# diharaw/hybrid-rendering

Measured on AMD Instinct MI355X. Metric: shadow Mrays/s over the fully denoised frame (1 spp trace + SVGF temporal + 4x a-trous), higher is better.
Workload: dtype f32; 1 GPU; 1920x1080 procedural Sponza-like (277968 tris) ray-traced shadows 1spp + SVGF denoise; trace_launch_order=heaviest tiles of the last frame first (csrc/tile_order.h), rays_per_frame_per_gpu=729543, pixels_per_gpu=2073600, bvh_nodes=23425

## Files before the change

### hybrid_rendering_amd/csrc/denoise_fast_shadows.hip

```cpp
#include "denoise_fast_common.h"
#include "mask_window.h"
#include "tile_order.h"

namespace {

#ifndef FT_SHADOWS_EU
#define FT_SHADOWS_EU 6
#endif
template <int GEO, int PATHS>
__global__ __launch_bounds__(64 * FT_WAVES, FT_SHADOWS_EU) void kf_shadows_temporal(TemporalArgs a)
{
    if (geo_apron_rides<64 * FT_WAVES>(a.apron)) return;
    if (tile_order_rides<64 * FT_WAVES>(a.sort)) return;
    const uint2 BLK = block_xy<0>();
    __shared__ uint32_t s_mask[FT_WAVES][1][18];
    __shared__ MaskRows s_rows[FT_WAVES];
    const int  lane = threadIdx.x & 63, wave = threadIdx.x >> 6;
    const int  txr = BLK.x * FT_WAVES + wave;
    const bool tile_ok = txr < a.tiles_x;
    const int  tx = tile_ok ? txr : 0, ty = (int)BLK.y + a.tile_y0;
    const int  lx = lane & 7, ly = lane >> 3;
    const int  x = tx * 8 + lx, y = ty * 8 + ly;
    const bool in_image = tile_ok && x < a.w && y < a.h && y >= a.y0 && y < a.y1;
    const bool edge     = tile_ok && (x >= a.w || y >= a.h);
// ... 213 lines not shown
                const uint32_t so = (uint32_t)(py * a.w + px);
                const uint32_t s  = fm::ld<uint32_t>(a.in.p, so * 4u);
                const uint2    nd = fm::ld<uint2>(a.nd, so * 8u);
                sum.add(ek, cnz, cv, nz_of(nd.x, nd.y), s, kk, true);
            }
        result = sum.finish(a.power);
    }
    *outp = result;
    if (out2p) *out2p = result;
    return 1;
}

template <int STEP, bool N32>
__global__ __launch_bounds__(256) void kf_shadows_atrous(AtrousArgs a)
{
    (void)shadows_atrous_body<STEP, N32>(a);
}

template <int STEP>
__global__ __launch_bounds__(256) void kf_shadows_atrous_timeline(AtrousArgs a, unsigned long long* timeline)
{
    const AtrousTimeline tl;
    const int live = shadows_atrous_body<STEP, true>(a);
    tl.exit(timeline, live);
}


template <int STEP, bool N32>
__global__ __launch_bounds__(256) void kf_shadows_atrous_lds(AtrousArgs a)
{
    const uint2 BLK = block_xy<0>();
    constexpr int TW = 32 + 2 * STEP, TH = 8 + 2 * STEP;
    __shared__ uint32_t s_in[TH * TW];
    __shared__ float4   s_nz[TH * TW];
    const int lx = threadIdx.x & 31, ly = threadIdx.x >> 5;
    const int bx0 = (int)BLK.x * 32, by0 = a.y0 + (int)BLK.y * 8;
    if (bx0 >= a.w) return;
    const int x = bx0 + lx, y = by0 + ly;
    const bool inside = x < a.w && y < a.y1;
    const uint32_t cls = inside ? a.tile_class[(size_t)(y >> 3) * a.tiles_x + (x >> 3)] : 0u;
    if (__syncthreads_or((int)cls))
    {
        const int ry0 = a.y0 > 0 ? a.y0 : 0, ry1 = a.y1 < a.h ? a.y1 : a.h;
        ShadowsStageBatch<(TH * TW + 255) / 256, TW, TH * TW> batch;
        batch.load(a, bx0 - STEP, by0 - STEP, ry0, ry1);
        __builtin_amdgcn_sched_barrier(0);
        batch.store(s_in, s_nz);
        __syncthreads();
    }
    if (!inside) return;
    const uint32_t o = (uint32_t)(y * a.w + x);
    uint32_t* outp  = reinterpret_cast<uint32_t*>(reinterpret_cast<char*>(a.out) + o * 4u);
    uint32_t* out2p = a.out2 ? reinterpret_cast<uint32_t*>(reinterpret_cast<char*>(a.out2) + o * 4u) : nullptr;
    if (!cls)
    {
        *outp = 0u;
        if (out2p) *out2p = 0u;
        return;
    }
    const int      ci     = (ly + STEP) * TW + (lx + STEP);
    const uint32_t result = shadows_filter<true>(StagedTaps { s_in, s_nz, TW, ci, TW, ci, STEP }, [&] { return edge_setup(a.sigma_depth, a.phi_normal, N32); }, a.phi_visibility, a.power);
    *outp = result;
    if (out2p) *out2p = result;
}

template <int TH, bool N32>
HR_DEV int shadows_atrous01_body(const AtrousArgs& a, uint32_t* out_first2, float power1)
{
    const uint2 BLK = block_xy<0>();
    constexpr int AW = 38, AH = TH + 6, BW = 36, BH = TH + 4;
    __shared__ uint32_t s_in[AH * AW];
    __shared__ float4   s_nz[AH * AW];
    __shared__ uint32_t s_mid[BH * BW];
    const int bx0 = (int)BLK.x * 32, by0 = a.y0 + (int)BLK.y * TH;
    if (bx0 >= a.w) return 0;
    const int ry0 = a.y0 > 0 ? a.y0 : 0, ry1 = a.y1 < a.h ? a.y1 : a.h;
    uint32_t any_cls = 0u;
    {
        const uint32_t cols = a.tiles_x - (bx0 >> 3) >= 4 ? 0xffffffffu : (1u << ((a.tiles_x - (bx0 >> 3)) * 8)) - 1u;
#pragma unroll
        for (int r = 0; r < TH / 8; r++)
        {
            const bool      row  = by0 + 8 * r < ry1;
            const uint32_t  tb   = (uint32_t)((by0 >> 3) + (row ? r : 0)) * (uint32_t)a.tiles_x + (uint32_t)(bx0 >> 3);
            const uint32_t* tc   = reinterpret_cast<const uint32_t*>(a.tile_class) + (tb >> 2);
            const uint32_t  cls4 = (uint32_t)(((uint64_t)tc[0] | ((uint64_t)tc[1] << 32)) >> ((tb & 3u) * 8u));
            any_cls |= row ? (cls4 & cols) : 0u;
        }
    }
    if (!any_cls)
    {
        for (int j = threadIdx.x; j < TH * 32; j += 256)
        {
            const int x = bx0 + (j & 31), y = by0 + (j >> 5);
            if (x >= a.w || y >= a.y1) continue;
            const uint32_t o = (uint32_t)(y * a.w + x);
            a.out[o] = 0u;
            if (a.out2) a.out2[o] = 0u;
            if (out_first2) out_first2[o] = 0u;
        }
        return 0;
    }
    ShadowsStageBatch<(AH * AW + 255) / 256, AW, AH * AW> batch;
    batch.load(a, bx0 - 3, by0 - 3, ry0, ry1);
    __builtin_amdgcn_sched_barrier(0);
    batch.store(s_in, s_nz);
    __syncthreads();
    const EdgeK ek = edge_setup(a.sigma_depth, a.phi_normal, N32);
    auto filter = [&](const uint32_t* img, int IW, int vi, int ci, int D, float power) -> uint32_t {
        return shadows_filter<true>(StagedTaps { img, s_nz, IW, vi, AW, ci, D }, [&] { return ek; }, a.phi_visibility, power);
    };
    for (int j = threadIdx.x; j < BH * BW; j += 256)
    {
        const int  cy = j / BW, cx = j - cy * BW;
        const int  gx = bx0 - 2 + cx, gy = by0 - 2 + cy;
        const bool res = gx >= 0 && gx < a.w && gy >= ry0 && gy < ry1;
        uint32_t   r = 0u;
        if (res && a.tile_class[(size_t)(gy >> 3) * a.tiles_x + (gx >> 3)])
        {
            const int ci = (cy + 1) * AW + cx + 1;
            r = filter(s_in, AW, ci, ci, 1, 0.0f);
        }
        s_mid[j] = r;
        if (out_first2 && res && cx >= 2 && cx < 34 && cy >= 2 && cy < 2 + TH && gy < a.y1) out_first2[(uint32_t)(gy * a.w + gx)] = r;
    }
    __syncthreads();
    for (int j = threadIdx.x; j < TH * 32; j += 256)
    {
        const int lx = j & 31, ly = j >> 5, x = bx0 + lx, y = by0 + ly;
        if (x >= a.w || y >= a.y1) continue;
        const uint32_t o = (uint32_t)(y * a.w + x);
        uint32_t r = 0u;
        if (a.tile_class[(size_t)(y >> 3) * a.tiles_x + (x >> 3)]) r = filter(s_mid, BW, (ly + 2) * BW + lx + 2, (ly + 3) * AW + lx + 3, 2, power1);
        a.out[o] = r;
        if (a.out2) a.out2[o] = r;
    }
    return 1;
}

template <int TH, bool N32>
__global__ __launch_bounds__(256) void kf_shadows_atrous01(AtrousArgs a, uint32_t* out_first2, float power1)
{
    (void)shadows_atrous01_body<TH, N32>(a, out_first2, power1);
}

template <int TH>
__global__ __launch_bounds__(256) void kf_shadows_atrous01_timeline(AtrousArgs a, uint32_t* out_first2, float power1, unsigned long long* timeline)
{
    const AtrousTimeline tl;
    const int live = shadows_atrous01_body<TH, true>(a, out_first2, power1);
    tl.exit(timeline, live);
}

}

namespace hr {

void launch_shadows_temporal_fast(const TemporalArgs& a_, int n_tiles, hipStream_t st)
{
    TemporalArgs a = a_;
    const dim3 grid = grid_with_apron(grid_with_sort(a.sort, grid_cols(cdiv(a.tiles_x, FT_WAVES), 4), a.tiles_y), a.apron, 64 * FT_WAVES);
    if (!a.geo_hist) hipLaunchKernelGGL((kf_shadows_temporal<0, 0>), grid, dim3(64 * FT_WAVES), 0, st, a);
    else if ((a.paths & TP_PAIRS) && a.w >= 2) hipLaunchKernelGGL((kf_shadows_temporal<1, TP_PAIRS>), grid, dim3(64 * FT_WAVES), 0, st, a);
    else hipLaunchKernelGGL((kf_shadows_temporal<1, 0>), grid, dim3(64 * FT_WAVES), 0, st, a);
}

void launch_shadows_atrous_fast(const AtrousArgs& a, hipStream_t st, unsigned long long* timeline)
{
    const dim3 grid(grid_cols(cdiv(a.w, 32), a.step >= 4 ? 0 : 7), cdiv(a.y1 - a.y0, 8));
    const bool n32 = a.phi_normal == 32.0f;
    if (timeline && n32 && a.radius == 1 && (a.step == 4 || a.step == 8))
    {
        if (a.step == 4) hipLaunchKernelGGL((kf_shadows_atrous_timeline<4>), grid, dim3(256), 0, st, a, timeline);
        else hipLaunchKernelGGL((kf_shadows_atrous_timeline<8>), grid, dim3(256), 0, st, a, timeline);
        return;
    }
#define HR_LAUNCH_ATROUS(K, S) \
    do { if (n32) hipLaunchKernelGGL((K<S, true>), grid, dim3(256), 0, st, a); else hipLaunchKernelGGL((K<S, false>), grid, dim3(256), 0, st, a); } while (0)
    if (a.radius == 1 && a.step == 1) HR_LAUNCH_ATROUS(kf_shadows_atrous_lds, 1);
    else if (a.radius == 1 && a.step == 2) HR_LAUNCH_ATROUS(kf_shadows_atrous_lds, 2);
    else if (a.radius == 1 && a.step == 4) HR_LAUNCH_ATROUS(kf_shadows_atrous, 4);
    else if (a.radius == 1 && a.step == 8) HR_LAUNCH_ATROUS(kf_shadows_atrous, 8);
    else HR_LAUNCH_ATROUS(kf_shadows_atrous, 0);
#undef HR_LAUNCH_ATROUS
}

#ifndef FT_ATROUS01_TH
#define FT_ATROUS01_TH 16
#endif
bool launch_shadows_atrous01_fast(const AtrousArgs& a, uint32_t* out_first2, float power1, hipStream_t st, int lds_pad, unsigned long long* timeline)
{
    if (a.radius != 1 || a.step != 1) return false;
    const dim3   grid(grid_cols(cdiv(a.w, 32), 7), cdiv(a.y1 - a.y0, FT_ATROUS01_TH));
    const size_t pad = lds_pad > 0 ? (size_t)lds_pad : 0;
    if (a.phi_normal != 32.0f) hipLaunchKernelGGL((kf_shadows_atrous01<FT_ATROUS01_TH, false>), grid, dim3(256), pad, st, a, out_first2, power1);
    else if (timeline) hipLaunchKernelGGL((kf_shadows_atrous01_timeline<FT_ATROUS01_TH>), grid, dim3(256), pad, st, a, out_first2, power1, timeline);
    else hipLaunchKernelGGL((kf_shadows_atrous01<FT_ATROUS01_TH, true>), grid, dim3(256), pad, st, a, out_first2, power1);
    return true;
}

int shadows_atrous01_static_lds()
{
    hipFuncAttributes fa;
    if (hipFuncGetAttributes(&fa, reinterpret_cast<const void*>(&kf_shadows_atrous01<FT_ATROUS01_TH, true>)) != hipSuccess) { (void)hipGetLastError(); return -1; }
    return (int)fa.sharedSizeBytes;
}
int shadows_atrous_max_workgroups(const AtrousArgs& a)
{
    return (cdiv(a.w, 32) + 8) * cdiv(a.y1 - a.y0, 8);
}

}
```

### hybrid_rendering_amd/csrc/pass_args.h

```cpp
#pragma once
#include "reproject.h"
#include "shading.h"
#include "upsample.h"

namespace hr {

struct TileSortArgs
{
    const uint16_t* cost;
    uint32_t*       order;
    int             n, groups;
    int             row0;
    int             min_spread;
};

struct GeoApronArgs
{
    const void* gb2;
    const void* gb3;
    void*       out;
    int         w, a0, a1, b0, b1;
    int         row0;
};

struct TemporalArgs
{
    float           vpi[16];
    const uint32_t* mask;
    int             mw, mh;
    ImgRGBA16F      gb2, gb3, pgb2, pgb3;
    ImgR32F         depth, pdepth;
    ImgRG16F        hist;
    ImgRGBA16F      hist_moments;
    uint32_t*       out;
    uint2*          out_moments;
    uint8_t*        tile_class;
    float4*         nd;
    const void*     geo_hist;
    int             w, h, y0, y1;
    int             tiles_x, tiles_y, tile_y0;
    float           alpha, moments_alpha;
    int             debug_skip_reproject;
    uint32_t*       apron_flag;
    int             band_y0, band_y1;
    TileSortArgs    sort;
    GeoApronArgs    apron;
    int             paths;
};

enum TemporalPaths : int
{
    TP_PAIRS = 1,
    TP_ALL   = 1
};

struct AtrousArgs
{
    ImgRG16F       in;
    const float4*  nd;
    const uint8_t* tile_class;
    uint32_t*      out;
    uint32_t*      out2;
    int            w, h, y0, y1, tiles_x;
    int            radius, step;
    float          phi_visibility, phi_normal, sigma_depth, power;
};

struct AOTemporalArgs
{
    float           vpi[16];
    const uint32_t* mask;
    int             mw, mh, spp;
    ImgRGBA16F      gb2, gb3, pgb2, pgb3;
    ImgR32F         depth, pdepth;
    ImgR16F         hist, hist_len;
    uint16_t*       out;
    uint16_t*       out_len;
    uint8_t*        tile_class;
    const void*     geo_hist;
    void*           geo_out;
    int             geo_band;
    int             w, h, y0, y1;
    int             tiles_x, tiles_y, tile_y0;
    float           alpha;
    uint32_t*       apron_flag;
    int             band_y0, band_y1;
    TileSortArgs    sort;
};

struct AOBlurArgs
{
    ImgR16F        in;
    ImgR32F        depth;
    ImgRGBA16F     gb2;
    const uint8_t* tile_class;
    uint16_t*      out;
    float          zbp[4];
    int            w, h, y0, y1, tiles_x;
    int            dx, dy, radius;
};

struct ReflTemporalArgs
{
    float       vpi[16], pvp[16];
    float       cam[3];
    ImgRGBA16F  in, gb2, gb3, pgb2, pgb3, hist, hist_moments;
    ImgR32F     depth, pdepth;
    uint2*      out;
    uint2*      out_moments;
    uint8_t*    tile_class;
    const void* geo_hist;
    void*       geo_out;
    int         w, h, y0, y1, tiles_x;
    float       alpha, moments_alpha;
    int         approximate_with_ddgi, moving;
    uint32_t*   apron_flag;
    int         band_y0, band_y1;
    TileSortArgs sort;
};

struct ReflAtrousArgs
{
    ImgRGBA16F     in, gb2, gb3;
    ImgR32F        depth;
    const void*    geo;
    const uint8_t* tile_class;
    uint2*         out;
    uint2*         out2;
    int            w, h, y0, y1, tiles_x, radius, step;
    float          phi_color, phi_normal, sigma_depth;
    int            approximate_with_ddgi;
};

struct DDGISampleArgs
{
    DDGIU        d;
    float        vpi[16];
    float        cam[3];
    const float* depth;
    const uint2* gb2;
    AtlasRGBA    irr;
    AtlasRG      dep;
    uint2*       out;
    int          w, h, y0, y1;
    float        gi_intensity;
};

void launch_shadows_temporal_fast(const TemporalArgs& a, int n_tiles, hipStream_t st);
void launch_shadows_atrous_fast(const AtrousArgs& a, hipStream_t st, unsigned long long* timeline = nullptr);
bool launch_shadows_atrous01_fast(const AtrousArgs& a, uint32_t* out_first2, float power1, hipStream_t st, int lds_pad = 0, unsigned long long* timeline = nullptr);
int  shadows_atrous01_static_lds();
int  shadows_atrous_max_workgroups(const AtrousArgs& a);
void launch_ao_temporal_fast(const AOTemporalArgs& a, int n_tiles, hipStream_t st);
void launch_ao_blur_fast(const AOBlurArgs& a, hipStream_t st);
bool launch_ao_blur_xy_fast(const AOBlurArgs& a, hipStream_t st);
void launch_refl_temporal_fast(const ReflTemporalArgs& a, hipStream_t st);
void launch_refl_atrous_fast(const ReflAtrousArgs& a, hipStream_t st);
bool launch_refl_atrous01_fast(const ReflAtrousArgs& a, uint2* out_first2, hipStream_t st);
void launch_ddgi_sample_fast(const DDGISampleArgs& a, hipStream_t st);
void launch_upsample_fast(const UpsampleArgs& a, hipStream_t st);

}
```

### hybrid_rendering_amd/csrc/shadows.hip

```cpp
#include "hr_internal.h"
#include "reproject.h"
#include "traverse.h"
#include "traverse2.h"
#include "shading.h"
#include "cutout_host.h"
#include "upsample.h"
#include "pass_args.h"
#include "tile_order.h"
#include "pass_core.h"

using namespace hr;

struct TraceArgs
{
    float           vpi[16];
    hr_light        light;
    const float*    depth;
    const uint2*    gb2;
    const uint8_t*  sobol;
    const uint8_t*  sr;
    uint32_t*       mask;
    uint16_t*       ray_slots;
    const Node8*    nodes;
    const TriGPU*   tris;
// ... 200 lines not shown
            {
                float sv = max2(mean - mean * mean, 0.0f);
                float sd = hr_sqrt(sv);
                hv       = clamp1(hv, mean - 0.5f * sd, mean + 0.5f * sd);
            }
            const float al = success ? max2(a.alpha, __fdiv_rn(1.0f, hlen)) : 1.0f;
            const float am = success ? max2(a.moments_alpha, __fdiv_rn(1.0f, hlen)) : 1.0f;
            m0      = visibility;
            m1      = m0 * m0;
            m0      = mix1(hm[0], m0, am);
            m1      = mix1(hm[1], m1, am);
            out_var = max2(0.0f, m1 - m0 * m0);
            out_v   = mix1(hv, visibility, al);
            flag    = out_v > 0.0f;
        }
        if (in_image)
        {
            a.out_moments[pix] = make_uint2(pack_h2(m0, m1), pack_h2(hlen, 0.0f));
            a.nd[pix]  = make_float4(cn.x, cn.y, cn.z, h2f_hi(cg3.y));
            a.out[pix] = pack_h2(out_v, out_var);
        }
    }
    if (a.apron_flag && __ballot(apron_miss) && lane == 0) atomicOr(a.apron_flag, 1u);
    const unsigned long long any = __ballot(flag);
    if (lane == 0) a.tile_class[(size_t)ty * a.tiles_x + tx] = any ? 1 : 0;
}


template <bool FAST>
HR_DEV float edge_weight(float cd, float sd, float phi_z, f3 cn, f3 sn, float phi_n, float cl, float sl, const DivBy& phi_l)
{
    const float dz = -fabsf(cd - sd);
    const float wZ = det_exp(FAST ? dz : __fdiv_rn(dz, phi_z));
    const float dn = clamp1(dot3(cn, sn), 0.0f, 1.0f);
    float wN;
    if (FAST) { float b = dn * dn; b = b * b; b = b * b; b = b * b; wN = b * b; }
    else wN = det_pow_auto(dn, phi_n);
    const float wL = div_by(fabsf(cl - sl), phi_l);
    return det_exp((0.0f - max2(wL, 0.0f)) - max2(wZ, 0.0f)) * wN;
}

template <int RADIUS, bool FAST>
__global__ __launch_bounds__(256) void k_shadows_atrous(AtrousArgs a)
{
    const int x = blockIdx.x * 32 + (threadIdx.x & 31);
    const int y = a.y0 + blockIdx.y * 8 + (threadIdx.x >> 5);
    if (x >= a.w || y >= a.y1) return;
    const size_t o = (size_t)y * a.w + x;
    if (!a.tile_class[(size_t)(y >> 3) * a.tiles_x + (x >> 3)])
    {
        a.out[o] = 0u;
        if (a.out2) a.out2[o] = 0u;
        return;
    }
    const uint32_t c  = a.in.p[o];
    uint32_t t_in[8];
    float4   t_nd[8];
    bool     t_ok[8];
    if (RADIUS == 1)
    {
#pragma unroll
        for (int t = 0; t < 8; t++)
        {
            const int k = t < 4 ? t : t + 1, xx = k % 3 - 1, yy = k / 3 - 1;
            const int px = x + xx * a.step, py = y + yy * a.step;
            t_ok[t] = px >= 0 && py >= 0 && px < a.w && py < a.h;
            const bool res = t_ok[t] && py >= a.y0 && py < a.y1;
            t_in[t] = res ? a.in.p[(size_t)py * a.w + px] : 0u;
            t_nd[t] = res ? a.nd[(size_t)py * a.w + px] : make_float4(0.0f, 0.0f, 0.0f, 0.0f);
        }
    }
    const float    cv = h2f_lo(c);
    float var = 0.0f;
#pragma unroll
    for (int yy = -1; yy <= 1; yy++)
#pragma unroll
        for (int xx = -1; xx <= 1; xx++)
        {
            const float k = (xx == 0 ? (yy == 0 ? 0.25f : 0.125f) : (yy == 0 ? 0.125f : 0.0625f));
            var += h2f_hi(a.in.raw(x + xx, y + yy)) * k;
        }
    const float4 cnd = a.nd[o];
    const float center_depth = cnd.w;
    uint32_t    result;
    if (center_depth < 0.0f) result = c;
    else
    {
        const f3    cn    = mk3(cnd.x, cnd.y, cnd.z);
        const DivBy phi_v = div_prepare(a.phi_visibility * hr_sqrt(max2(0.0f, 1e-10f + var)));
        float sum_w = 1.0f, sum_v = cv, sum_var = h2f_hi(c);
        if (RADIUS == 1)
        {
            float w8[8];
#pragma unroll
            for (int t = 0; t < 8; t++)
                w8[t] = edge_weight<FAST>(center_depth, t_nd[t].w, a.sigma_depth, cn, mk3(t_nd[t].x, t_nd[t].y, t_nd[t].z), a.phi_normal, cv, h2f_lo(t_in[t]), phi_v);
#pragma unroll
            for (int t = 0; t < 8; t++)
            {
                if (!t_ok[t]) continue;
                const int   k = t < 4 ? t : t + 1, xx = k % 3 - 1, yy = k / 3 - 1;
                const float kx = xx == 0 ? 1.0f : __fdiv_rn(2.0f, 3.0f), ky = yy == 0 ? 1.0f : __fdiv_rn(2.0f, 3.0f);
                const float sv = h2f_lo(t_in[t]);
                const float wv = w8[t] * (kx * ky);
                sum_w += wv;
                sum_v += wv * sv;
                sum_var += (wv * wv) * h2f_hi(t_in[t]);
            }
        }
        else
        {
        const int R = RADIUS >= 0 ? RADIUS : a.radius;
        for (int yy = -R; yy <= R; yy++)
            for (int xx = -R; xx <= R; xx++)
            {
                const int px = x + xx * a.step, py = y + yy * a.step;
                if (px < 0 || py < 0 || px >= a.w || py >= a.h || (xx == 0 && yy == 0)) continue;
                const int   axx = xx < 0 ? -xx : xx, ayy = yy < 0 ? -yy : yy;
                const float kx = axx == 0 ? 1.0f : (axx == 1 ? __fdiv_rn(2.0f, 3.0f) : __fdiv_rn(1.0f, 6.0f));
                const float ky = ayy == 0 ? 1.0f : (ayy == 1 ? __fdiv_rn(2.0f, 3.0f) : __fdiv_rn(1.0f, 6.0f));
                const uint32_t s  = a.in.raw(px, py);
                const float4   snd = (py >= a.y0 && py < a.y1) ? a.nd[(size_t)py * a.w + px] : make_float4(0.0f, 0.0f, 0.0f, 0.0f);
                const float    sv = h2f_lo(s);
                const f3       sn = mk3(snd.x, snd.y, snd.z);
                const float    w  = edge_weight<FAST>(center_depth, snd.w, a.sigma_depth, cn, sn, a.phi_normal, cv, sv, phi_v);
                const float    wv = w * (kx * ky);
                sum_w += wv;
                sum_v += wv * sv;
                sum_var += (wv * wv) * h2f_hi(s);
            }
        }
        float ov = __fdiv_rn(sum_v, sum_w), ovar = __fdiv_rn(sum_var, sum_w * sum_w);
        if (a.power != 0.0f) ov = det_pow_auto(ov, a.power);
        result = pack_h2(ov, ovar);
    }
    a.out[o] = result;
    if (a.out2) a.out2[o] = result;
}

struct hr_shadows : PassCore
{
    DevBuf  mask, temporal_out, moments[2], prev_image, atrous[2], nd, occluder;
    int     temporal_paths = TP_ALL;
    bool    occluder_cache = true;
    int     read_idx = 0;
    int     last_ping_pong = 0;
    int           latched_exact = -1;
    int           dbg_only_tx = -1, dbg_only_ty = -1;
    bool          dbg_skip_traversal = false, dbg_skip_reproject = false, dbg_timeline_stats = false;
    std::string   dbg_timeline;
    uint64_t      last_wave_max_steps = 0;
    void*         nd_cur = nullptr;
    int           atrous01_pad = 0;
    std::string   dbg_atrous_timeline;
};

#ifndef FT_ATROUS01_RESIDENT
#define FT_ATROUS01_RESIDENT 6
#endif
#ifndef HR_ATROUS01_REGIONS_PER_SLOT
#define HR_ATROUS01_REGIONS_PER_SLOT 4
#endif
#define HR_LDS_GRANULE 1280

struct AtrousTimelineDump
{
    DevBuf buf;
    unsigned long long* ptr() const { return (unsigned long long*)buf.p; }
    hr_status begin(const std::string& prefix, const AtrousArgs& a)
    {
        if (prefix.empty()) return HR_OK;
        return buf.alloc((size_t)shadows_atrous_max_workgroups(a) * 4 * 32);
    }
    hr_status end(const std::string& prefix, const char* tag, hipStream_t st)
    {
        if (!buf.p) return HR_OK;
        HR_HIP(hipStreamSynchronize(st));
        std::vector<unsigned long long> host(buf.bytes / 8);
        HR_HIP(hipMemcpy(host.data(), buf.p, buf.bytes, hipMemcpyDeviceToHost));
        if (FILE* f = fopen((prefix + "." + tag).c_str(), "wb")) { fwrite(host.data(), 8, host.size(), f); fclose(f); }
        return HR_OK;
    }
};

bool hr::profiling_enabled(const hr_shadows* p) { return p && p->prof.enabled; }

extern "C" {

void hr_shadows_default_params(hr_shadows_params* p)
{
    p->denoise = 1; p->bias = 0.5f; p->alpha = 0.01f; p->moments_alpha = 0.2f; p->phi_visibility = 10.0f;
    p->phi_normal = 32.0f; p->sigma_depth = 1.0f; p->power = 1.2f; p->radius = 1; p->filter_iterations = 4; p->feedback_iteration = 1;
    p->exact = 1;
}

hr_status hr_shadows_create(hr_ctx* ctx, int32_t full_width, int32_t full_height, hr_scale scale, const hr_band* band, hr_shadows** out)
{
    hr_shadows* p = nullptr;
    hr_status   s = pass_new(&p, ctx, full_width, full_height, scale, band, out, BandRule::Shadows, "shadows");
    if (s != HR_OK) return s;
    if (const char* e = getenv("HR_DEBUG_ONLY_TILE")) sscanf(e, "%d,%d", &p->dbg_only_tx, &p->dbg_only_ty);
    if (const char* e = getenv("HR_SHADOW_CACHE")) p->occluder_cache = atoi(e) != 0;
    if (const char* e = getenv("HR_TEMPORAL_PAIRS")) p->temporal_paths = atoi(e) != 0 ? (p->temporal_paths | TP_PAIRS) : (p->temporal_paths & ~TP_PAIRS);
    p->tile_order.min_spread = HR_ORDER_COHERENT_SPREAD;
    p->dbg_skip_traversal = getenv("HR_DEBUG_SKIP_TRAVERSAL") != nullptr;
    p->dbg_skip_reproject = getenv("HR_DEBUG_SKIP_REPROJECT") != nullptr;
    p->dbg_timeline_stats = getenv("HR_DEBUG_TIMELINE_STATS") != nullptr;
    if (const char* e = getenv("HR_DEBUG_TIMELINE")) p->dbg_timeline = e;
    if (const char* e = getenv("HR_DEBUG_ATROUS_TIMELINE")) p->dbg_atrous_timeline = e;
    {
        int resident = FT_ATROUS01_RESIDENT;
        if (const char* e = getenv("HR_ATROUS01_RESIDENT")) resident = atoi(e);
        hipDeviceProp_t prop;
        if (resident >= 3 && hipGetDeviceProperties(&prop, ctx->device) == hipSuccess)
        {
            const int own = shadows_atrous01_static_lds(), regions = cdiv(p->w, 32) * cdiv(p->y1 - p->y0, 16);
            if (regions > HR_ATROUS01_REGIONS_PER_SLOT * resident * prop.multiProcessorCount) resident = 0;
            if (own >= 0) p->atrous01_pad = atrous_resident_pad((int)prop.maxSharedMemoryPerMultiProcessor, own, resident, HR_LDS_GRANULE);
            if (own + p->atrous01_pad > (int)prop.sharedMemPerBlock) p->atrous01_pad = 0;
        }
    }
    const size_t px = (size_t)p->w * p->h;
    HR_PASS_ALLOC(mask, (size_t)p->mw * p->mh * 4)
    HR_PASS_ALLOC(temporal_out, px * 4)
    HR_PASS_ALLOC(moments[0], px * 8)
    HR_PASS_ALLOC(moments[1], px * 8)
    HR_PASS_ALLOC(prev_image, px * 4)
    HR_PASS_ALLOC(atrous[0], px * 4)
    HR_PASS_ALLOC(atrous[1], px * 4)
    HR_PASS_ALLOC(upsample, (size_t)full_width * full_height * 2)
    HR_PASS_ALLOC(tile_class, (((size_t)p->tiles_x * p->tiles_y + 3) & ~(size_t)3) + 8)
    HR_PASS_ALLOC(nd, px * 16)
    HR_PASS_ALLOC(counters, 64)
    HR_PASS_ALLOC(ray_slots, (size_t)p->tiles_x * p->tiles_y * 2)
    HR_PASS_ALLOC(occluder, px * 4)
    if ((s = p->tile_order.init(p->resident_tiles())) != HR_OK) { delete p; return s; }
    HR_HIP(hipMemset(p->occluder.p, 0xff, p->occluder.bytes));
    HR_HIP(hipMemset(p->counters.p, 0, 64));
    HR_HIP(hipMemset(p->ray_slots.p, 0, p->ray_slots.bytes));
    HR_HIP(hipMemset(p->mask.p, 0, p->mask.bytes));
    HR_HIP(hipMemset(p->tile_class.p, 0, p->tile_class.bytes));
    *out = p;
    return HR_OK;
}

hr_status hr_shadows_destroy(hr_shadows* p) { return pass_destroy(p); }
hr_status hr_shadows_reset_history(hr_shadows* p) { return pass_reset_history(p); }
hr_status hr_shadows_history_apron_exceeded(hr_shadows* p, int32_t* exceeded) { return pass_history_apron_exceeded(p, exceeded); }
hr_status hr_shadows_set_profiling(hr_shadows* p, int32_t enable) { return pass_set_profiling(p, enable); }
hr_status hr_shadows_get_stage_times(hr_shadows* p, hr_stage_times* out) { return pass_get_stage_times(p, out); }
hr_status hr_shadows_ray_count(hr_shadows* p, uint64_t* rays) { return pass_ray_count<uint16_t>(p, rays); }
hr_status hr_shadows_launch_order(hr_shadows* p, uint32_t* out, int32_t* n_tiles) { return pass_launch_order(p, out, n_tiles); }

hr_status hr_shadows_tile_ray_counts(hr_shadows* p, uint16_t* out, int32_t* tiles_x, int32_t* tiles_y)
{
    HR_CHECK_ARG(p);
    if (tiles_x) *tiles_x = p->tiles_x;
    if (tiles_y) *tiles_y = p->tiles_y;
    if (!out) return HR_OK;
    HR_HIP(hipStreamSynchronize(p->last_stream));
    HR_HIP(hipMemcpy(out, p->ray_slots.p, (size_t)p->tiles_x * p->tiles_y * 2, hipMemcpyDeviceToHost));
    return HR_OK;
}

hr_status hr_shadows_ray_trace(hr_shadows* p, const hr_scene* scene, const hr_frame_inputs* in, const hr_shadows_params* prm, void* stream_)
{
    HR_CHECK_ARG(p && scene && in && prm);
    hr_status s = check_inputs(p, in, false);
    if (s != HR_OK) return s;
    HR_CHECK_ARG(in->sobol && in->scrambling_ranking);
    HR_REJECT_SHARED_DEV(scene, "hr_shadows_ray_trace", p->want_stats || !p->dbg_timeline.empty() || p->dbg_skip_traversal || p->dbg_only_tx >= 0);
    HR_REJECT_CUTOUT(scene, HR_RAY_SHADOW, "hr_shadows_ray_trace", p->want_stats || !p->dbg_timeline.empty() || p->dbg_skip_traversal || p->dbg_only_tx >= 0);
    const bool       cutout = cutout_on(scene, HR_RAY_SHADOW);
    const CutoutView cv = cutout ? cutout_view_of(scene) : CutoutView();
    hipStream_t st = (hipStream_t)stream_;
    p->last_stream = st;
    if (p->first_frame)
    {
        HR_HIP(hipMemsetAsync(p->prev_image.p, 0, p->prev_image.bytes, st));
        HR_HIP(hipMemsetAsync(p->moments[!in->ping_pong].p, 0, p->moments[0].bytes, st));
        p->first_frame = false;
    }
    TraceArgs a;
    for (int i = 0; i < 16; i++) a.vpi[i] = in->ubo.view_proj_inverse[i];
    a.light = in->ubo.light;
    a.depth = in->cur.depth; a.gb2 = (const uint2*)in->cur.gb2;
    a.sobol = in->sobol; a.sr = in->scrambling_ranking;
    a.mask = (uint32_t*)p->mask.p; a.ray_slots = (uint16_t*)p->ray_slots.p;
    a.nodes = (const Node8*)scene->nodes.p; a.tris = (const TriGPU*)scene->tris.p; a.inst = (const InstanceShared*)scene->inst_shared.p; a.cull = cull_of(scene, HR_RAY_SHADOW);
    a.stats = nullptr;
    a.timeline = nullptr;
    a.w = p->w; a.h = p->h; a.y0 = p->y0; a.y1 = p->y1; a.mw = p->mw;
    a.tile_y0 = p->tile_y0(); a.tiles_x = p->tiles_x; a.tiles_y = p->resident_tiles_y();
    a.bias = prm->bias; a.num_frames = in->num_frames;
    a.occluder = p->occluder_cache ? (uint32_t*)p->occluder.p : nullptr;
    a.n_tri_refs = (uint32_t)(scene->tris.bytes / sizeof(TriGPU));
    const int n_tiles = a.tiles_x * a.tiles_y;
    const int n_slots = n_tiles;
    a.debug_only_tx = p->dbg_only_tx; a.debug_only_ty = p->dbg_only_ty;
    a.debug_skip_traversal = p->dbg_skip_traversal ? 1 : 0;
    if ((s = p->tile_order.flush(st)) != HR_OK) return s;
    a.order = p->tile_order.order_arg(n_tiles); a.cost = p->tile_order.cost_arg(n_tiles);
    const uint64_t px = (uint64_t)p->w * (p->y1 - p->y0);
    if (p->want_stats)
    {
        a.cost = nullptr;
        HR_HIP(hipMemsetAsync((char*)p->counters.p + 16, 0, 24, st));
        a.stats = (unsigned long long*)((char*)p->counters.p + 16);
        hipLaunchKernelGGL(k_shadows_trace<true>, dim3(cdiv(n_slots, TRACE_WAVES)), dim3(64 * TRACE_WAVES), 0, st, a, cv);
        HR_HIP(hipGetLastError());
        return HR_OK;
    }
    if (!p->dbg_timeline.empty())
    {
        const char* tl = p->dbg_timeline.c_str();
        DevBuf buf;
        hr_status bs = buf.alloc((size_t)n_tiles * 32);
        if (bs != HR_OK) return bs;
        a.timeline = (unsigned long long*)buf.p;
        if (p->dbg_timeline_stats) hipLaunchKernelGGL(k_shadows_trace<true>, dim3(cdiv(n_slots, TRACE_WAVES)), dim3(64 * TRACE_WAVES), 0, st, a, cv);
        else hipLaunchKernelGGL(k_shadows_trace<false>, dim3(cdiv(n_slots, TRACE_WAVES)), dim3(64 * TRACE_WAVES), 0, st, a, cv);
        HR_HIP(hipStreamSynchronize(st));
        std::vector<unsigned long long> host((size_t)n_tiles * 4);
        HR_HIP(hipMemcpy(host.data(), buf.p, host.size() * 8, hipMemcpyDeviceToHost));
        if (FILE* f = fopen(tl, "wb")) { fwrite(host.data(), 8, host.size(), f); fclose(f); }
        a.timeline = nullptr;
    }
    int ev = p->prof.begin("ray_trace", st, px * 12 + px / 8);
    const auto kernel = scene->shared ? (cutout ? k_shadows_trace<false, true, true> : k_shadows_trace<false, true>)
                                      : (cutout ? k_shadows_trace<false, false, true> : k_shadows_trace<false>);
    hipLaunchKernelGGL(kernel, dim3(cdiv(n_slots, TRACE_WAVES)), dim3(64 * TRACE_WAVES), 0, st, a, cv);
    p->prof.end(ev, st);
    HR_HIP(hipGetLastError());
    if (a.cost && (s = p->tile_order.traced(n_tiles, st)) != HR_OK) return s;
    return HR_OK;
}

hr_status hr_shadows_trace_divergence(hr_shadows* p, uint64_t* wave_max_steps)
{
    HR_CHECK_ARG(p && wave_max_steps);
    *wave_max_steps = p->last_wave_max_steps;
    return HR_OK;
}

static hr_status shadows_trace_stats_impl(hr_shadows* p, const hr_scene* scene, const hr_frame_inputs* in, const hr_shadows_params* prm, uint64_t* out3, void* stream, bool walk_only)
{
    HR_CHECK_ARG(p && out3);
    const bool cache = p->occluder_cache;
    p->want_stats = true;
    if (walk_only) p->occluder_cache = false;
    hr_status s = hr_shadows_ray_trace(p, scene, in, prm, stream);
    p->want_stats = false;
    p->occluder_cache = cache;
    if (s != HR_OK) return s;
    HR_HIP(hipStreamSynchronize((hipStream_t)stream));
    uint64_t host[5];
    HR_HIP(hipMemcpy(host, p->counters.p, 40, hipMemcpyDeviceToHost));
    hr_status rs = hr_shadows_ray_count(p, &out3[0]);
    if (rs != HR_OK) return rs;
    out3[1] = host[2]; out3[2] = host[3];
    p->last_wave_max_steps = host[4];
    return HR_OK;
}

hr_status hr_shadows_trace_stats(hr_shadows* p, const hr_scene* scene, const hr_frame_inputs* in, const hr_shadows_params* prm, uint64_t* out3, void* stream)
{
    return shadows_trace_stats_impl(p, scene, in, prm, out3, stream, true);
}

hr_status hr_shadows_trace_stats_timed(hr_shadows* p, const hr_scene* scene, const hr_frame_inputs* in, const hr_shadows_params* prm, uint64_t* out3, void* stream)
{
    return shadows_trace_stats_impl(p, scene, in, prm, out3, stream, false);
}

hr_status hr_shadows_temporal(hr_shadows* p, const hr_frame_inputs* in, const hr_shadows_params* prm, void* stream_)
{
    HR_CHECK_ARG(p && in && prm);
    hr_status s = check_inputs(p, in, true);
    if (s != HR_OK) return s;
    hipStream_t st = (hipStream_t)stream_;
    p->last_stream = st;
    p->latched_exact = prm->exact ? 1 : 0;
    TemporalArgs a;
    for (int i = 0; i < 16; i++) a.vpi[i] = in->ubo.view_proj_inverse[i];
    a.mask = (const uint32_t*)p->mask.p; a.mw = p->mw; a.mh = p->mh;
    const int w = p->w, y0 = p->y0, y1 = p->y1, ry0 = p->ry0, ry1 = p->ry1;
    a.gb2  = ImgRGBA16F { (const uint2*)in->cur.gb2, w, ry0, ry1 };
    a.gb3  = ImgRGBA16F { (const uint2*)in->cur.gb3, w, ry0, ry1 };
    a.pgb2 = ImgRGBA16F { (const uint2*)in->prev.gb2, w, ry0, ry1 };
    a.pgb3 = ImgRGBA16F { (const uint2*)in->prev.gb3, w, ry0, ry1 };
    a.depth  = ImgR32F { in->cur.depth, w, ry0, ry1 };
    a.pdepth = ImgR32F { in->prev.depth, w, ry0, ry1 };
    a.hist         = ImgRG16F { (const uint32_t*)p->prev_image.p, w, ry0, ry1 };
    a.hist_moments = ImgRGBA16F { (const uint2*)p->moments[!in->ping_pong].p, w, ry0, ry1 };
    a.out = (uint32_t*)p->temporal_out.p; a.out_moments = (uint2*)p->moments[in->ping_pong ? 1 : 0].p;
    a.tile_class = (uint8_t*)p->tile_class.p;
    a.nd = (float4*)p->nd.p;
    a.geo_hist = nullptr;
    a.apron = GeoApronArgs { nullptr, nullptr, nullptr, 0, 0, 0, 0, 0, -1 };
    if (!prm->exact)
    {
        const size_t half = (size_t)p->w * p->h * 8;
        const GeoRecords::Step g = p->records.advance(in->cur.gb2, in->cur.gb3, in->prev.gb2, in->prev.gb3, p->first_frame);
        if (g.read >= 0) a.geo_hist = (const char*)p->nd.p + (size_t)g.read * half;
        a.nd = (float4*)((char*)p->nd.p + (size_t)g.write * half);
        if (p->records.history && (ry0 < y0 || ry1 > y1))
            a.apron = GeoApronArgs { in->cur.gb2, in->cur.gb3, a.nd, w, ry0, y0, y1, ry1, -1 };
        if (g.require_failed) return geo_require_error("hr_shadows_temporal");
    }
    else p->records.invalidate();
    p->nd_cur = a.nd;
    a.w = w; a.h = p->h; a.y0 = y0; a.y1 = y1;
    a.tile_y0 = p->tile_y0(); a.tiles_x = p->tiles_x; a.tiles_y = p->resident_tiles_y();
    a.alpha = prm->alpha; a.moments_alpha = prm->moments_alpha;
    a.debug_skip_reproject = p->dbg_skip_reproject ? 1 : 0;
    a.apron_flag = p->apron_flag();
    a.band_y0 = p->band_y0; a.band_y1 = p->band_y1;
    a.paths = p->temporal_paths;
    p->last_ping_pong = in->ping_pong ? 1 : 0;
    const uint64_t px = (uint64_t)w * (y1 - y0);
    int ev = p->prof.begin("temporal_accumulation", st, px * 64 + px / 8);
    a.sort = TileSortArgs { nullptr, nullptr, 0, 0, 0, 0 };
    if (prm->exact) hipLaunchKernelGGL(k_shadows_temporal, dim3(cdiv(a.tiles_x * a.tiles_y, TEMPORAL_WAVES)), dim3(64 * TEMPORAL_WAVES), 0, st, a);
    else
    {
        a.sort = p->tile_order.ride();
        launch_shadows_temporal_fast(a, a.tiles_x * a.tiles_y, st);
    }
    p->prof.end(ev, st);
    HR_HIP(hipGetLastError());
    return HR_OK;
}

static hr_status check_mode(hr_shadows* p, const hr_shadows_params* prm);

hr_status hr_shadows_atrous_iteration(hr_shadows* p, const hr_frame_inputs* in, const hr_shadows_params* prm, int32_t i, void* stream_)
{
    HR_CHECK_ARG(p && in && prm && i >= 0 && i < prm->filter_iterations && prm->filter_iterations <= 8 && prm->radius >= 0 && prm->radius <= 2);
    hr_status s = check_inputs(p, in, false);
    if (s != HR_OK) return s;
    if ((s = check_mode(p, prm)) != HR_OK) return s;
    hipStream_t st = (hipStream_t)stream_;
    p->last_stream = st;
    const int read_idx = i & 1, write_idx = (i & 1) ^ 1;
    AtrousArgs a;
    const int w = p->w, y0 = p->y0, y1 = p->y1;
    a.in  = ImgRG16F { (const uint32_t*)(i == 0 ? p->temporal_out.p : p->atrous[read_idx].p), w, y0, y1 };
    a.nd = (const float4*)(p->nd_cur ? p->nd_cur : p->nd.p);
    a.tile_class = (const uint8_t*)p->tile_class.p;
    a.out  = (uint32_t*)p->atrous[write_idx].p;
    a.out2 = (prm->feedback_iteration == i) ? (uint32_t*)p->prev_image.p : nullptr;
    a.w = w; a.h = p->h; a.y0 = y0; a.y1 = y1; a.tiles_x = p->tiles_x;
    a.radius = prm->radius; a.step = 1 << i;
    a.phi_visibility = prm->phi_visibility; a.phi_normal = prm->phi_normal; a.sigma_depth = prm->sigma_depth;
    a.power = (i == prm->filter_iterations - 1) ? prm->power : 0.0f;
    p->read_idx = write_idx;
    static const char* names[8] = { "atrous_0", "atrous_1", "atrous_2", "atrous_3", "atrous_4", "atrous_5", "atrous_6", "atrous_7" };
    const uint64_t px = (uint64_t)w * (y1 - y0);
    int ev = p->prof.begin(names[i], st, px * 24 + (a.out2 ? px * 4 : 0));
    const dim3 grid(cdiv(w, 32), cdiv(y1 - y0, 8));
    const bool fast = (prm->phi_normal == 32.0f && prm->sigma_depth == 1.0f);
    AtrousTimelineDump tl;
    if (!prm->exact && p->fuse && prm->radius == 1 && (i == 2 || i == 3) && (s = tl.begin(p->dbg_atrous_timeline, a)) != HR_OK) return s;
    if (!prm->exact) launch_shadows_atrous_fast(a, st, tl.ptr());
    else if (prm->radius == 1 && fast) hipLaunchKernelGGL((k_shadows_atrous<1, true>), grid, dim3(256), 0, st, a);
    else if (prm->radius == 1) hipLaunchKernelGGL((k_shadows_atrous<1, false>), grid, dim3(256), 0, st, a);
    else hipLaunchKernelGGL((k_shadows_atrous<-1, false>), grid, dim3(256), 0, st, a);
    p->prof.end(ev, st);
    HR_HIP(hipGetLastError());
    if ((s = tl.end(p->dbg_atrous_timeline, i == 2 ? "atrous4" : "atrous8", st)) != HR_OK) return s;
    return HR_OK;
}

static hr_status check_mode(hr_shadows* p, const hr_shadows_params* prm)
{
    if (p->latched_exact >= 0 && p->latched_exact != (prm->exact ? 1 : 0))
    {
        set_last_error("hr_shadows: params.exact changed between the temporal and the a-trous stage of one frame");
        return HR_ERR_INVALID_ARG;
    }
    return HR_OK;
}

static hr_status shadows_atrous01(hr_shadows* p, const hr_frame_inputs* in, const hr_shadows_params* prm, void* stream_, bool* done)
{
    hr_status s = check_inputs(p, in, false);
    if (s != HR_OK) return s;
    if ((s = check_mode(p, prm)) != HR_OK) return s;
    hipStream_t st = (hipStream_t)stream_;
    p->last_stream = st;
    AtrousArgs a;
    const int w = p->w, y0 = p->y0, y1 = p->y1;
    a.in  = ImgRG16F { (const uint32_t*)p->temporal_out.p, w, y0, y1 };
    a.nd = (const float4*)(p->nd_cur ? p->nd_cur : p->nd.p);
    a.tile_class = (const uint8_t*)p->tile_class.p;
    a.out  = (uint32_t*)p->atrous[0].p;
    a.out2 = (prm->feedback_iteration == 1) ? (uint32_t*)p->prev_image.p : nullptr;
    uint32_t* first2 = (prm->feedback_iteration == 0) ? (uint32_t*)p->prev_image.p : nullptr;
    a.w = w; a.h = p->h; a.y0 = y0; a.y1 = y1; a.tiles_x = p->tiles_x;
    a.radius = prm->radius; a.step = 1;
    a.phi_visibility = prm->phi_visibility; a.phi_normal = prm->phi_normal; a.sigma_depth = prm->sigma_depth;
    a.power = 0.0f;
    const uint64_t px = (uint64_t)w * (y1 - y0);
    AtrousTimelineDump tl;
    if ((s = tl.begin(p->dbg_atrous_timeline, a)) != HR_OK) return s;
    int ev = p->prof.begin("atrous_01", st, px * 16 + ((a.out2 || first2) ? px * 4 : 0));
    *done = launch_shadows_atrous01_fast(a, first2, prm->filter_iterations == 2 ? prm->power : 0.0f, st, p->atrous01_pad, tl.ptr());
    p->prof.end(ev, st);
    if ((s = tl.end(p->dbg_atrous_timeline, "atrous01", st)) != HR_OK) return s;
    if (*done) p->read_idx = 0;
    HR_HIP(hipGetLastError());
    return HR_OK;
}

hr_status hr_shadows_upsample(hr_shadows* p, const hr_frame_inputs* in, const hr_shadows_params* prm, void* stream)
{
    HR_CHECK_ARG(p && in && prm);
    const uint64_t PX = (uint64_t)p->full_w * p->full_h, px = (uint64_t)p->w * p->h;
    return pass_upsample(p, in, prm->exact != 0, p->atrous[p->read_idx].p, 2, 1, 0.0f, 0.0f, PX * 18 + px * 20, stream);
}

hr_status hr_shadows_denoise(hr_shadows* p, const hr_frame_inputs* in, const hr_shadows_params* prm, void* stream)
{
    HR_CHECK_ARG(p && in && prm);
    p->last_denoise = prm->denoise != 0;
    if (!prm->denoise) return HR_OK;
    hr_status s;
    if ((s = hr_shadows_temporal(p, in, prm, stream)) != HR_OK) return s;
    {
        HR_SCOPED_SAMPLE("A-Trous Filter");
        bool fused = false;
        if (!prm->exact && p->fuse && prm->filter_iterations >= 2 && prm->filter_iterations <= 8 && prm->radius == 1 &&
            (s = shadows_atrous01(p, in, prm, stream, &fused)) != HR_OK) return s;
        for (int i = fused ? 2 : 0; i < prm->filter_iterations; i++)
            if ((s = hr_shadows_atrous_iteration(p, in, prm, i, stream)) != HR_OK) return s;
    }
    if (p->scale != 0 && (s = hr_shadows_upsample(p, in, prm, stream)) != HR_OK) return s;
    return HR_OK;
}

hr_status hr_shadows_render(hr_shadows* p, const hr_scene* scene, const hr_frame_inputs* in, const hr_shadows_params* prm, void* stream)
{
    HR_SCOPED_SAMPLE("Ray Traced Shadows");
    HR_CHECK_ARG(p && scene && in && prm);
    HR_HIP(hipSetDevice(p->ctx->device));
    p->prof.begin_frame();
    p->last_denoise = prm->denoise != 0;
    hr_status s = hr_shadows_ray_trace(p, scene, in, prm, stream);
    if (s != HR_OK) return s;
    return hr_shadows_denoise(p, in, prm, stream);
}

hr_status hr_shadows_image(hr_shadows* p, int32_t which, hr_image_view* v)
{
    HR_CHECK_ARG(p && v);
    switch (which)
    {
        case 0: fill_view(v, p->mask.p, p->mw, p->mh, 4, HR_FORMAT_R32_UINT); break;
        case 1: fill_view(v, p->temporal_out.p, p->w, p->h, 4, HR_FORMAT_RG16F); break;
        case 2: fill_view(v, p->moments[0].p, p->w, p->h, 8, HR_FORMAT_RGBA16F); break;
        case 3: fill_view(v, p->moments[1].p, p->w, p->h, 8, HR_FORMAT_RGBA16F); break;
        case 4: fill_view(v, p->prev_image.p, p->w, p->h, 4, HR_FORMAT_RG16F); break;
        case 5: fill_view(v, p->atrous[0].p, p->w, p->h, 4, HR_FORMAT_RG16F); break;
        case 6: fill_view(v, p->atrous[1].p, p->w, p->h, 4, HR_FORMAT_RG16F); break;
        case 7: fill_view(v, p->upsample.p, p->full_w, p->full_h, 2, HR_FORMAT_R16F); break;
        case 8: fill_view(v, p->tile_class.p, p->tiles_x, p->tiles_y, 1, (hr_format)0); break;
        case 9:
            if (!p->nd_cur || p->latched_exact != 0) { set_last_error("hr_shadows_image(9): no geometry records (parity mode, or no temporal stage yet)"); return HR_ERR_INVALID_ARG; }
            fill_view(v, p->nd_cur, p->w, p->h, 8, HR_FORMAT_RGBA16F); break;
        default: set_last_error("hr_shadows_image: unknown image index"); return HR_ERR_INVALID_ARG;
    }
    return HR_OK;
}

hr_status hr_shadows_output(hr_shadows* p, hr_output_kind kind, hr_image_view* v)
{
    HR_CHECK_ARG(p && v);
    if (!p->last_denoise || kind == HR_OUTPUT_RAY_TRACE) return hr_shadows_image(p, 0, v);
    if (kind == HR_OUTPUT_TEMPORAL_ACCUMULATION) return hr_shadows_image(p, 1, v);
    if (kind == HR_OUTPUT_ATROUS || p->scale == 0) return hr_shadows_image(p, 5 + p->read_idx, v);
    return hr_shadows_image(p, 7, v);
}

}
```

Baseline: 4880 Mrays/s.

## Stage a-trous step-4/8 tiles with apron into LDS before filtering

Adds a new a-trous kernel for tap distances 4 and 8. Each block first loads its tile plus a STEP-wide apron of visibility and normal/depth into shared memory, then filters from LDS. Blocks whose tiles are all empty take an early exit and write zeros. Tile height (8 or 16 rows) is picked from the region count versus CU count, and the kernel is on by default for the step-4 pass only. The apron adds overhead, especially at step 8, and the large LDS footprint can lower occupancy.

New measurement: 4909 Mrays/s, median of 6. Within noise of the previous version (+0.6%).

```diff
diff --git a/hybrid_rendering_amd/csrc/denoise_fast_shadows.hip b/hybrid_rendering_amd/csrc/denoise_fast_shadows.hip
--- a/hybrid_rendering_amd/csrc/denoise_fast_shadows.hip
+++ b/hybrid_rendering_amd/csrc/denoise_fast_shadows.hip
@@ -389,6 +389,68 @@
     tl.exit(timeline, live);
 }
 
+template <int STEP, int TH, bool N32>
+__global__ __launch_bounds__(256) void kf_shadows_atrous_staged(AtrousArgs a)
+{
+    static_assert((STEP == 4 || STEP == 8) && (TH == 8 || TH == 16 || TH == 32), "tap distance 4 / 8, 1 / 2 / 4 tile rows");
+    const uint2 BLK = block_xy<0>();
+    constexpr int AW = 32 + 2 * STEP, AH = TH + 2 * STEP, ROWS = TH / 8;
+    __shared__ uint32_t s_in[AH * AW];
+    __shared__ float4   s_nz[AH * AW];
+    const int bx0 = (int)BLK.x * 32, by0 = a.y0 + (int)BLK.y * TH;
+    if (bx0 >= a.w) return;
+    const int ry0 = a.y0 > 0 ? a.y0 : 0, ry1 = a.y1 < a.h ? a.y1 : a.h;
+    uint32_t cls[ROWS], any_cls = 0u;
+    {
+        const uint32_t cols = a.tiles_x - (bx0 >> 3) >= 4 ? 0xffffffffu : (1u << ((a.tiles_x - (bx0 >> 3)) * 8)) - 1u;
+#pragma unroll
+        for (int r = 0; r < ROWS; r++)
+        {
+            const bool      row  = by0 + 8 * r < ry1;
+            const uint32_t  tb   = (uint32_t)((by0 >> 3) + (row ? r : 0)) * (uint32_t)a.tiles_x + (uint32_t)(bx0 >> 3);
+            const uint32_t* tc   = reinterpret_cast<const uint32_t*>(a.tile_class) + (tb >> 2);
+            const uint32_t  cls4 = (uint32_t)(((uint64_t)tc[0] | ((uint64_t)tc[1] << 32)) >> ((tb & 3u) * 8u));
+            cls[r] = row ? (cls4 & cols) : 0u;
+            any_cls |= cls[r];
+        }
+    }
+    const int lx = threadIdx.x & 31, ly = threadIdx.x >> 5;
+    if (!any_cls)
+    {
+#pragma unroll
+        for (int r = 0; r < ROWS; r++)
+        {
+            const int x = bx0 + lx, y = by0 + 8 * r + ly;
+            if (x >= a.w || y >= a.y1) continue;
+            const uint32_t o = (uint32_t)(y * a.w + x);
+            a.out[o] = 0u;
+            if (a.out2) a.out2[o] = 0u;
+        }
+        return;
+    }
+    ShadowsStageBatch<(AH * AW + 255) / 256, AW, AH * AW> batch;
+    batch.load(a, bx0 - STEP, by0 - STEP, ry0, ry1);
+    __builtin_amdgcn_sched_barrier(0);
+    batch.store(s_in, s_nz);
+    __syncthreads();
+    const EdgeK ek = edge_setup(a.sigma_depth, a.phi_normal, N32);
+#pragma unroll
+    for (int r = 0; r < ROWS; r++)
+    {
+        const int x = bx0 + lx, y = by0 + 8 * r + ly;
+        if (x >= a.w || y >= a.y1) continue;
+        const uint32_t o = (uint32_t)(y * a.w + x);
+        uint32_t result = 0u;
+        if ((cls[r] >> ((lx >> 3) * 8)) & 0xffu)
+        {
+            const int ci = (8 * r + ly + STEP) * AW + lx + STEP;
+            result = shadows_filter<true>(StagedTaps { s_in, s_nz, AW, ci, AW, ci, STEP }, [&] { return ek; }, a.phi_visibility, a.power);
+        }
+        a.out[o] = result;
+        if (a.out2) a.out2[o] = result;
+    }
+}
+
 }
 
 namespace hr {
@@ -402,7 +464,7 @@
     else hipLaunchKernelGGL((kf_shadows_temporal<1, 0>), grid, dim3(64 * FT_WAVES), 0, st, a);
 }
 
-void launch_shadows_atrous_fast(const AtrousArgs& a, hipStream_t st, unsigned long long* timeline)
+void launch_shadows_atrous_fast(const AtrousArgs& a, hipStream_t st, unsigned long long* timeline, int staged_th)
 {
     const dim3 grid(grid_cols(cdiv(a.w, 32), a.step >= 4 ? 0 : 7), cdiv(a.y1 - a.y0, 8));
     const bool n32 = a.phi_normal == 32.0f;
@@ -410,6 +472,18 @@
     {
         if (a.step == 4) hipLaunchKernelGGL((kf_shadows_atrous_timeline<4>), grid, dim3(256), 0, st, a, timeline);
         else hipLaunchKernelGGL((kf_shadows_atrous_timeline<8>), grid, dim3(256), 0, st, a, timeline);
+        return;
+    }
+    if (staged_th && a.radius == 1 && (a.step == 4 || a.step == 8))
+    {
+        const dim3 sgrid(grid.x, cdiv(a.y1 - a.y0, a.step == 4 ? staged_th : 16));
+#define HR_LAUNCH_STAGED(S, T) \
+        do { if (n32) hipLaunchKernelGGL((kf_shadows_atrous_staged<S, T, true>), sgrid, dim3(256), 0, st, a); \
+             else hipLaunchKernelGGL((kf_shadows_atrous_staged<S, T, false>), sgrid, dim3(256), 0, st, a); } while (0)
+        if (a.step == 8) HR_LAUNCH_STAGED(8, 16);
+        else if (staged_th == 8) HR_LAUNCH_STAGED(4, 8);
+        else HR_LAUNCH_STAGED(4, 16);
+#undef HR_LAUNCH_STAGED
         return;
     }
 #define HR_LAUNCH_ATROUS(K, S) \
diff --git a/hybrid_rendering_amd/csrc/pass_args.h b/hybrid_rendering_amd/csrc/pass_args.h
--- a/hybrid_rendering_amd/csrc/pass_args.h
+++ b/hybrid_rendering_amd/csrc/pass_args.h
@@ -147,7 +147,7 @@
 };
 
 void launch_shadows_temporal_fast(const TemporalArgs& a, int n_tiles, hipStream_t st);
-void launch_shadows_atrous_fast(const AtrousArgs& a, hipStream_t st, unsigned long long* timeline = nullptr);
+void launch_shadows_atrous_fast(const AtrousArgs& a, hipStream_t st, unsigned long long* timeline = nullptr, int staged_th = 0);
 bool launch_shadows_atrous01_fast(const AtrousArgs& a, uint32_t* out_first2, float power1, hipStream_t st, int lds_pad = 0, unsigned long long* timeline = nullptr);
 int  shadows_atrous01_static_lds();
 int  shadows_atrous_max_workgroups(const AtrousArgs& a);
diff --git a/hybrid_rendering_amd/csrc/shadows.hip b/hybrid_rendering_amd/csrc/shadows.hip
--- a/hybrid_rendering_amd/csrc/shadows.hip
+++ b/hybrid_rendering_amd/csrc/shadows.hip
@@ -376,6 +376,7 @@
     uint64_t      last_wave_max_steps = 0;
     void*         nd_cur = nullptr;
     int           atrous01_pad = 0;
+    int           atrous_staged_th[2] = { 0, 0 };
     std::string   dbg_atrous_timeline;
 };
 
@@ -386,6 +387,12 @@
 #define HR_ATROUS01_REGIONS_PER_SLOT 4
 #endif
 #define HR_LDS_GRANULE 1280
+#ifndef FT_ATROUS_STAGED
+#define FT_ATROUS_STAGED 1
+#endif
+#ifndef HR_ATROUS_STAGED_TALL_REGIONS
+#define HR_ATROUS_STAGED_TALL_REGIONS 40
+#endif
 
 struct AtrousTimelineDump
 {
@@ -443,6 +450,19 @@
             if (own >= 0) p->atrous01_pad = atrous_resident_pad((int)prop.maxSharedMemoryPerMultiProcessor, own, resident, HR_LDS_GRANULE);
             if (own + p->atrous01_pad > (int)prop.sharedMemPerBlock) p->atrous01_pad = 0;
         }
+    }
+    {
+        int staged = FT_ATROUS_STAGED, th4 = 0;
+        if (const char* e = getenv("HR_ATROUS_STAGED")) staged = atoi(e);
+        if (const char* e = getenv("HR_ATROUS_STAGED_TH")) th4 = atoi(e);
+        if (th4 != 8 && th4 != 16)
+        {
+            hipDeviceProp_t prop;
+            const int cus = hipGetDeviceProperties(&prop, ctx->device) == hipSuccess ? prop.multiProcessorCount : 256;
+            th4 = cdiv(p->w, 32) * cdiv(p->y1 - p->y0, 16) > HR_ATROUS_STAGED_TALL_REGIONS * cus ? 16 : 8;
+        }
+        if (staged & 1) p->atrous_staged_th[0] = th4;
+        if (staged & 2) p->atrous_staged_th[1] = 16;
     }
     const size_t px = (size_t)p->w * p->h;
     HR_PASS_ALLOC(mask, (size_t)p->mw * p->mh * 4)
@@ -686,7 +706,8 @@
     const bool fast = (prm->phi_normal == 32.0f && prm->sigma_depth == 1.0f);
     AtrousTimelineDump tl;
     if (!prm->exact && p->fuse && prm->radius == 1 && (i == 2 || i == 3) && (s = tl.begin(p->dbg_atrous_timeline, a)) != HR_OK) return s;
-    if (!prm->exact) launch_shadows_atrous_fast(a, st, tl.ptr());
+    const int sk = (!prm->exact && p->fuse && prm->radius == 1 && (i == 2 || i == 3)) ? i - 2 : -1;
+    if (!prm->exact) launch_shadows_atrous_fast(a, st, tl.ptr(), sk >= 0 ? p->atrous_staged_th[sk] : 0);
     else if (prm->radius == 1 && fast) hipLaunchKernelGGL((k_shadows_atrous<1, true>), grid, dim3(256), 0, st, a);
     else if (prm->radius == 1) hipLaunchKernelGGL((k_shadows_atrous<1, false>), grid, dim3(256), 0, st, a);
     else hipLaunchKernelGGL((k_shadows_atrous<-1, false>), grid, dim3(256), 0, st, a);
```
